# liuQuan98/EYOC

Measured on AMD Instinct MI355X. Metric: registered pairs/sec (30k-voxel KITTI pairs), higher is better.
Workload: dtype f32 (split16 products: fp32 storage/accumulation, 3 fp16 MFMAs on hi/lo-split operands per product); 1 GPU; 64 synthetic 30 cm KITTI-shaped pairs per step per GPU (mean 29894 voxels/cloud, ResUNetBN2C random-init, 5000-point NN, RANSAC 4000000 hypotheses/pair, planted inlier ratio 0.3, spconv math split16); parallelism=pairs sharded over 1 GPU(s), steps_in_flight=2

## Files before the change

eyoc_amd/_lib.py:

```python
from __future__ import annotations

import ctypes as C
import os
import threading

_HERE = os.path.dirname(os.path.abspath(__file__))
LIB_PATH = os.environ.get("EYOC_HIP_LIB") or os.path.join(_HERE, "lib", "libeyoc_hip.so")

MAX_LEVELS = 4
MAP_S1, MAP_DOWN, MAP_UP = 0, 1, 2


class MapsInfo(C.Structure):
    _fields_ = [("n_levels", C.c_int32), ("rows", C.c_int32 * MAX_LEVELS),
                ("pairs_s1", C.c_int64 * MAX_LEVELS), ("pairs_down", C.c_int64 * MAX_LEVELS),
                ("pairs_up", C.c_int64 * MAX_LEVELS), ("pairs_conv1", C.c_int64)]


class ModelDesc(C.Structure):
    _fields_ = [("in_channels", C.c_int32), ("out_channels", C.c_int32), ("conv1_kernel_size", C.c_int32),
                ("normalize_feature", C.c_int32), ("channels", C.c_int32 * 5), ("tr_channels", C.c_int32 * 5),
                ("bn_eps", C.c_float), ("expanded", C.c_int32)]


# ... 121 lines not shown
    "eyoc_model_layer_ms": (_i, [_vp, C.POINTER(C.c_float)]),
    "eyoc_model_timing_slot": (_i, [_vp, _i]),
    "eyoc_bn_workspace_bytes": (_sz, [_i, _i]),
    "eyoc_bn_train_forward": (_i, [_vp, _vp, _i, _i, _i, _vp, _vp, C.c_float, _i, _vp, _i, _vp, _vp, _sz, _vp]),
    "eyoc_bn_train_forward_running": (_i, [_vp, _vp, _i, _i, _i, _vp, _vp, C.c_float, _i, _vp, _i, _vp, _vp, _vp, C.c_float, _vp, _sz, _vp]),
    "eyoc_bn_train_backward": (_i, [_vp, _vp, _i, _vp, _i, _vp, _i, _i, _i, _vp, _vp, C.c_float, _vp, _i, _vp, _vp, _vp, _sz, _vp]),
    "eyoc_maps_gather_window": (_i, [_vp, _vp, _i, _vp, _i, _vp, _vp]),
    "eyoc_maps_gather_window_internal": (_i, [_vp, _vp, _i, _vp, _i, _vp, _vp]),
    "eyoc_knn_prefilter": (_i, [_vp, _i]),
    "eyoc_spconv_select_up_kernel": (_i, [_vp, _i]),
    "eyoc_spconv_upc_min_rows": (_i, [_vp, _i]),
    "eyoc_spconv_upc_tile_rows": (_i, [_i, _i]),
    "eyoc_spconv_upc_bytes": (_sz, [_i]),
    "eyoc_spconv_upc_build": (_i, [_vp, _vp, _i, _vp, _vp, _vp]),
    "eyoc_spconv_upc": (_i, [_vp, _vp, _vp, _i, _i, _vp, _i, _i, _vp, _i, _vp, _i, _vp, _i, _i, _vp, _vp]),
    "eyoc_spconv_select_conv1_kernel": (_i, [_vp, _i]),
    "eyoc_knn1": (_i, [_vp, _vp, _vp, _i, C.POINTER(C.c_int32), C.POINTER(C.c_int32), _i, _i, _vp, _vp, _vp]),
    "eyoc_pdist": (_i, [_vp, _vp, _i, _vp, _i, _i, _i, _vp, _vp]),
    "eyoc_kabsch_batched": (_i, [_vp, _vp, _vp, _vp, _i, _i, _vp, _vp]),
    "eyoc_irls_quad": (_i, [_vp, _vp, _vp, _vp, _i, _i, _vp, _vp]),
    "eyoc_ransac": (_i, [_vp, _vp, _vp, _vp, _i, C.POINTER(RansacParams), _vp, _vp]),
    "eyoc_maps_select_orders": (_i, [_vp, _i, _i]),
    "eyoc_ransac_select_pruning": (_i, [_vp, _i]),
    "eyoc_registration_accept_degenerate": (_i, [_vp, _i]),
    "eyoc_ransac_transform_store": (_i, [_vp, _i]),
    "eyoc_ransac_workspace_bytes": (_sz, [_vp, _i, _i, _i, _sz]),
    "eyoc_ransac_batched_ws": (_i, [_vp, _vp, _vp, _vp, C.POINTER(C.c_int32), C.POINTER(C.c_int32), _i,
                                    C.POINTER(RansacParams), _vp, _vp, _sz, _vp]),
    "eyoc_ransac_batched": (_i, [_vp, _vp, _vp, _vp, C.POINTER(C.c_int32), C.POINTER(C.c_int32), _i,
                                 C.POINTER(RansacParams), _vp, _vp]),
    "eyoc_sc2pcr_workspace_bytes": (_sz, [_i, C.POINTER(Sc2pcrParams)]),
    "eyoc_sc2pcr": (_i, [_vp, _vp, _vp, _i, C.POINTER(Sc2pcrParams), _vp, _vp, _vp, _sz, _vp]),
    "eyoc_sc2pcr_batched_workspace_bytes": (_sz, [_i, C.POINTER(Sc2pcrParams)]),
    "eyoc_sc2pcr_batched_workspace_bytes_n": (_sz, [_i, _i, C.POINTER(Sc2pcrParams)]),
    "eyoc_sc2pcr_set_shortlist_cap": (_i, [_vp, _i]),
    "eyoc_sc2pcr_set_dense_threshold": (_i, [_vp, _i]),
    "eyoc_sc2pcr_select_kernels": (_i, [_vp, _i]),
    "eyoc_sc2pcr_workspace_layout": (_i, [_i, C.POINTER(Sc2pcrParams), C.POINTER(Sc2pcrLayout)]),
    "eyoc_sc2pcr_batched": (_i, [_vp, _vp, _vp, C.POINTER(C.c_int32), _i, C.POINTER(Sc2pcrParams), _vp, _vp, _i, _vp, _sz,
                                 _vp]),
    "eyoc_icp_workspace_bytes": (_sz, [_i, _i, _i]),
    "eyoc_icp_batched": (_i, [_vp, _vp, _vp, C.POINTER(C.c_int32), C.POINTER(C.c_int32), _i, _vp, C.POINTER(IcpParams), _vp, _vp,
                              _vp, _sz, _vp]),
    "eyoc_icp_correspondences": (_i, [_vp, _vp, _vp, C.POINTER(C.c_int32), C.POINTER(C.c_int32), _i, _vp, C.c_double, _vp, _vp,
                                      _vp, _vp, _sz, _vp]),
}
# ... 139 lines not shown
```

eyoc_amd/csrc/common.h:

```cpp
#pragma once
#include <hip/hip_runtime.h>

#include <cstdarg>
#include <cstdint>
#include <cstdio>
#include <cstring>
#include <string>
#include <vector>

#include "../../include/eyoc_hip.h"

namespace eyoc {

void set_error(const char* fmt, ...);

#define EYOC_CHECK_HIP(expr)                                                               \
  do {                                                                                     \
    hipError_t _e = (expr);                                                                \
    if (_e != hipSuccess) {                                                                \
      eyoc::set_error("%s failed: %s (%s:%d)", #expr, hipGetErrorString(_e), __FILE__,    \
                      __LINE__);                                                           \
      return EYOC_ERR_HIP;                                                                 \
    }                                                                                      \
  } while (0)
// ... 49 lines not shown
  struct Knobs {
    int maps_order_min_rows = 65536;
    int maps_window_shift = 18;
    int maps_s1_order = 1, maps_down_order = 0;
    int maps_internal_order = -1;
    int maps_lazy_tables = 1, maps_fused_levels = 1;
    int knn_prefilter = 1;
    int fuse_tail = 2;
    int spconv_kernel = -1;
    int split16_kernel = 1;
    int up_kernel = 2;
    int s1_wide = 1;
    int st128_wide = 1;
    int down_kernel = 1;
    int upc_min_rows = 1 << 17;
    int conv1_kernel = 1;
    int st_group = 1;
    int st_variant = 1;
    int st_split_below = 1024;
    int st_cg_local = 1;
    int st_ksplit = 1;
    int ransac_store = 1 << 20;
    int ransac_prune = 2;
    int accept_degenerate = 0;
  } knobs;
};
inline const eyoc_ctx::Knobs& knobs_of(const eyoc_ctx* ctx) {
  static const eyoc_ctx::Knobs defaults;
  return ctx ? ctx->knobs : defaults;
}

namespace eyoc {

constexpr unsigned long long KEY_EMPTY = 0xFFFFFFFFFFFFFFFFull;
constexpr int COORD_BIAS = 1 << 17;
constexpr int VAL_UNSET = 0x7F7F7F7F;

struct HashTable {
  unsigned long long* keys;
  int* vals;
  unsigned int mask;
};

__host__ __device__ inline unsigned long long pack_key(int b, int x, int y, int z) {
  return ((unsigned long long)(unsigned)b << 54) |
         ((unsigned long long)((unsigned)(x + COORD_BIAS) & 0x3FFFFu) << 36) |
// ... 69 lines not shown
```

eyoc_amd/csrc/ransac.hip:

```cpp
#include "pose_math.h"

using namespace eyoc;

namespace {

__device__ inline void sample_pair(unsigned long long base, unsigned long long ctr, unsigned int n, unsigned int& i0,
                                   unsigned int& i1) {
  unsigned long long x = base + ctr;
  x = (x ^ (x >> 30)) * 0xBF58476D1CE4E5B9ull;
  x = (x ^ (x >> 27)) * 0x94D049BB133111EBull;
  x = x ^ (x >> 31);
  i0 = __umulhi((unsigned int)x, n);
  i1 = __umulhi((unsigned int)(x >> 32), n);
}

constexpr int CHUNK = 64;
struct PairArgs {
  int s0[CHUNK], n[CHUNK], t0[CHUNK];
  int pair0;
  float* rec;
  unsigned int seed;
  int H;
  float edge_sim, max_dist;
  int* n_surv;
  int* surv;
  int* cnts;
  unsigned int* rmse;
  double* xf;
  int cap_t;
  float* rec_sorted;
  float* rr_sorted;
  int* bucket_end;
  double* pmax;
  int count_bound;
};

__global__ void k_gather_targets(const float* __restrict__ src, const float* __restrict__ tgt,
                                 const long long* __restrict__ corr, PairArgs a) {
  const int c = blockIdx.y;
  const int s0 = a.s0[c], n = a.n[c];
  float* rec = a.rec;
  const int i = blockIdx.x * blockDim.x + threadIdx.x;
  if (i >= n) return;
  const long long j = a.t0[c] + corr[s0 + i];
  float* r = rec + (size_t)(s0 + i) * 6;
  r[0] = src[3 * (size_t)(s0 + i)]; r[1] = src[3 * (size_t)(s0 + i) + 1]; r[2] = src[3 * (size_t)(s0 + i) + 2];
  r[3] = tgt[3 * j]; r[4] = tgt[3 * j + 1]; r[5] = tgt[3 * j + 2];
}

__device__ inline bool sample_and_check_edges(const float* __restrict__ rec, unsigned int n, unsigned long long base,
                                              unsigned int h, double edge_sim, double s[4][3], double q[4][3]) {
  unsigned int idx[4];
  sample_pair(base, 2ull * h, n, idx[0], idx[1]);
  sample_pair(base, 2ull * h + 1, n, idx[2], idx[3]);
#pragma unroll
  for (int j = 0; j < 4; ++j) {
    const float2* r = reinterpret_cast<const float2*>(rec + (size_t)idx[j] * 6);
// ... 147 lines not shown
  const int* __restrict__ cand = a.cnts + (size_t)c * a.H;
  int* surv = a.surv + (size_t)c * a.H;
  const double edge_sim = (double)a.edge_sim, max_dist = (double)a.max_dist;
  for (int i = blockIdx.x * 256 + threadIdx.x; i < ncand; i += gridDim.x * 256) {
    const int h = cand[i];
    double s[4][3], q[4][3], R[3][3], t[3];
    sample_and_check_edges(rec, (unsigned)n, base, (unsigned)h, edge_sim, s, q);
    if (!fit_and_check_distance(s, q, max_dist, R, t)) continue;
    const int slot = atomicAdd(cnt, 1);
    surv[slot] = h;
    if (slot < a.cap_t) {
      double* x = a.xf + ((size_t)c * a.cap_t + slot) * 12;
#pragma unroll
      for (int k = 0; k < 3; ++k) {
        x[3 * k] = R[k][0]; x[3 * k + 1] = R[k][1]; x[3 * k + 2] = R[k][2];
        x[9 + k] = t[k];
      }
    }
  }
}

__device__ inline double thr2_of(float max_dist) { return (double)max_dist * (double)max_dist; }

constexpr int NBUCKET = 64;

__global__ __launch_bounds__(256) void k_bucket(PairArgs a) {
  __shared__ int hist[NBUCKET], start[NBUCKET];
  __shared__ double red[4];
  const int c = blockIdx.x;
  const int s0 = a.s0[c], n = a.n[c];
  const float* __restrict__ rec = a.rec + (size_t)s0 * 6;
  float* __restrict__ out = a.rec_sorted + (size_t)s0 * 6;
  int* bend = a.bucket_end + c * (NBUCKET + 1);
  const int ns = a.n_surv[c * CNT_STRIDE];
  if (threadIdx.x < NBUCKET) hist[threadIdx.x] = 0;
  __syncthreads();
  const bool have_ref = ns > 0;
  double R[9] = {1, 0, 0, 0, 1, 0, 0, 0, 1}, t[3] = {0, 0, 0};
  if (have_ref) {
    const double* x = a.xf + (size_t)c * a.cap_t * 12;
#pragma unroll
    for (int i = 0; i < 9; ++i) R[i] = x[i];
    t[0] = x[9]; t[1] = x[10]; t[2] = x[11];
  }
  const double inv_w = 1.0 / (double)a.max_dist;
  double pm = 0.0;
  int bkt[32];
#pragma unroll
  for (int u = 0; u < 32; ++u) {
    const int i = u * 256 + (int)threadIdx.x;
    bkt[u] = -1;
    if (i < n) {
      const float2* r = reinterpret_cast<const float2*>(rec + (size_t)i * 6);
      const float2 p0 = r[0], p1 = r[1], p2 = r[2];
      const double x = p0.x, y = p0.y, z = p1.x;
      const double dx = fma(R[0], x, fma(R[1], y, fma(R[2], z, t[0] - (double)p1.y)));
      const double dy = fma(R[3], x, fma(R[4], y, fma(R[5], z, t[1] - (double)p2.x)));
      const double dz = fma(R[6], x, fma(R[7], y, fma(R[8], z, t[2] - (double)p2.y)));
      const double d = sqrt(fma(dx, dx, fma(dy, dy, dz * dz)));
      const double q = d * inv_w;
      int b = have_ref ? (q < (double)(NBUCKET - 1) ? (int)q : NBUCKET - 1) : 0;
      if (!(q == q)) b = NBUCKET - 1;
      bkt[u] = b;
      atomicAdd(&hist[b], 1);
      pm = fmax(pm, sqrt(fma(x, x, fma(y, y, z * z))));
    }
  }
#pragma unroll
  for (int d = 32; d >= 1; d >>= 1) pm = fmax(pm, __shfl_xor(pm, d, 64));
  if ((threadIdx.x & 63) == 0) red[threadIdx.x >> 6] = pm;
  __syncthreads();
  if (threadIdx.x == 0) {
    int acc = 0;
    for (int b = 0; b < NBUCKET; ++b) { start[b] = acc; acc += hist[b]; bend[b] = acc; }
    bend[NBUCKET] = n;
    a.pmax[c] = fmax(fmax(red[0], red[1]), fmax(red[2], red[3]));
  }
  __syncthreads();
#pragma unroll
  for (int u = 0; u < 32; ++u) {
    const int i = u * 256 + (int)threadIdx.x;
    if (bkt[u] >= 0) {
      const int pos = atomicAdd(&start[bkt[u]], 1);
      const float2* r = reinterpret_cast<const float2*>(rec + (size_t)i * 6);
      float2* w = reinterpret_cast<float2*>(out + (size_t)pos * 6);
      const float2 p0 = r[0], p1 = r[1], p2 = r[2];
      w[0] = p0; w[1] = p1; w[2] = p2;
      const double x = p0.x, y = p0.y, z = p1.x;
      const double dx = fma(R[0], x, fma(R[1], y, fma(R[2], z, t[0] - (double)p1.y)));
      const double dy = fma(R[3], x, fma(R[4], y, fma(R[5], z, t[1] - (double)p2.x)));
      const double dz = fma(R[6], x, fma(R[7], y, fma(R[8], z, t[2] - (double)p2.y)));
      reinterpret_cast<float4*>(a.rr_sorted)[(size_t)s0 + pos] = make_float4((float)dx, (float)dy, (float)dz, 0.f);
    }
  }
}

constexpr int PPL = 4;

__global__ __launch_bounds__(256) void k_count_fp64(PairArgs a, const double* __restrict__ xf_all, int pruned) {
  const int c = blockIdx.y;
  const int s0 = a.s0[c], n = a.n[c];
  const float* __restrict__ rec = (pruned ? a.rec_sorted : a.rec) + (size_t)s0 * 6;
  const int lane = threadIdx.x & 63;
  const int wave = __builtin_amdgcn_readfirstlane((int)(threadIdx.x >> 6));
  const int ns_all = a.n_surv[c * CNT_STRIDE];
  const int ns = ns_all < a.cap_t ? ns_all : a.cap_t;
  const double thr2 = thr2_of(a.max_dist);
  const double* __restrict__ xf = xf_all + (size_t)c * a.cap_t * 12;
  const int* __restrict__ bend = a.bucket_end + c * (NBUCKET + 1);
  int* cnts = a.cnts + (size_t)c * a.H;
  int G = 64;
  while (G > 8 && (ns + G - 1) / G < (int)gridDim.x * 4) G >>= 1;
  const int n_groups = (ns + G - 1) / G;
  int best = 0;
  for (int grp = blockIdx.x * 4 + wave; grp < n_groups; grp += gridDim.x * 4) {
    const int sbase = grp * G;
    const int gs = min(G, ns - sbase);
    int hi = 0;
    if (lane < gs) {
      hi = n;
      if (pruned) {
        const double* __restrict__ T = xf + (size_t)(sbase + lane) * 12;
        double fr = 0.0, dt = 0.0;
#pragma unroll
        for (int i = 0; i < 9; ++i) { const double e = T[i] - xf[i]; fr = fma(e, e, fr); }
#pragma unroll
        for (int i = 9; i < 12; ++i) { const double e = T[i] - xf[i]; dt = fma(e, e, dt); }
        const double delta = (sqrt(fr) * a.pmax[c] + sqrt(dt)) * (1.0 + 1e-9) + 1e-9;
        const double q = ((double)a.max_dist + delta) / (double)a.max_dist;
        const int b = q < (double)(NBUCKET - 2) ? (int)q + 1 : NBUCKET;
        hi = bend[b < NBUCKET ? b : NBUCKET];
      }
    }
    int hi_max = hi;
#pragma unroll
    for (int d = 32; d >= 1; d >>= 1) hi_max = max(hi_max, __shfl_xor(hi_max, d, 64));
    hi_max = __builtin_amdgcn_readfirstlane(hi_max);
    int mycnt = 0;
    for (int i0 = 0; i0 < hi_max; i0 += 64 * PPL) {
      double x[PPL], y[PPL], z[PPL], qx[PPL], qy[PPL], qz[PPL];
#pragma unroll
      for (int u = 0; u < PPL; ++u) {
        const int i = i0 + u * 64 + lane;
        if (i < n) {
          const float2* r = reinterpret_cast<const float2*>(rec + (size_t)i * 6);
          const float2 p0 = r[0], p1 = r[1], p2 = r[2];
          x[u] = p0.x; y[u] = p0.y; z[u] = p1.x; qx[u] = p1.y; qy[u] = p2.x; qz[u] = p2.y;
        } else {
          x[u] = y[u] = z[u] = 0.0; qx[u] = qy[u] = qz[u] = 1e18;
        }
// ... 5 lines not shown
        const double r00 = T[0], r01 = T[1], r02 = T[2], r10 = T[3], r11 = T[4], r12 = T[5], r20 = T[6], r21 = T[7], r22 = T[8];
        const double t0 = T[9], t1 = T[10], t2 = T[11];
        int csum = 0;
#pragma unroll
        for (int u = 0; u < PPL; ++u) {
          const double dx = fma(r00, x[u], fma(r01, y[u], fma(r02, z[u], t0 - qx[u])));
          const double dy = fma(r10, x[u], fma(r11, y[u], fma(r12, z[u], t1 - qy[u])));
          const double dz = fma(r20, x[u], fma(r21, y[u], fma(r22, z[u], t2 - qz[u])));
          const double d2 = fma(dx, dx, fma(dy, dy, dz * dz));
          csum += __popcll(__ballot(d2 < thr2));
        }
        mycnt += lane == s ? csum : 0;
      }
    }
    if (lane < gs) cnts[sbase + lane] = mycnt;
    best = mycnt > best ? mycnt : best;
  }
#pragma unroll
  for (int d = 32; d >= 1; d >>= 1) best = max(best, __shfl_xor(best, d, 64));
  if (lane == 0 && best > 0) atomicMax(a.n_surv + c * CNT_STRIDE + 1, best);
}

typedef float f32x2 __attribute__((ext_vector_type(2)));
constexpr int PKP = 4;
constexpr int KC_RECORDS = 64 * 2 * PKP;

__device__ inline bool inlier_fp64(const float* __restrict__ rec, int i, const double* __restrict__ T, double thr2) {
  const float2* r = reinterpret_cast<const float2*>(rec + (size_t)i * 6);
  const float2 p0 = r[0], p1 = r[1], p2 = r[2];
  const double x = p0.x, y = p0.y, z = p1.x;
  const double dx = fma(T[0], x, fma(T[1], y, fma(T[2], z, T[9] - (double)p1.y)));
  const double dy = fma(T[3], x, fma(T[4], y, fma(T[5], z, T[10] - (double)p2.x)));
  const double dz = fma(T[6], x, fma(T[7], y, fma(T[8], z, T[11] - (double)p2.y)));
  return fma(dx, dx, fma(dy, dy, dz * dz)) < thr2;
}

__global__ __launch_bounds__(256) __attribute__((amdgpu_waves_per_eu(5, 5))) void k_count(PairArgs a, const double* __restrict__ xf_all) {
  __shared__ float4 deltas[4][64][3];
  const int c = blockIdx.y;
  const int s0 = a.s0[c], n = a.n[c];
  const float* __restrict__ rec = a.rec_sorted + (size_t)s0 * 6;
  const float4* __restrict__ rr = reinterpret_cast<const float4*>(a.rr_sorted) + s0;
  const int lane = threadIdx.x & 63;
  const int wave = __builtin_amdgcn_readfirstlane((int)(threadIdx.x >> 6));
  const int ns_all = a.n_surv[c * CNT_STRIDE];
  const int ns = ns_all < a.cap_t ? ns_all : a.cap_t;
  const double thr = (double)a.max_dist, thr2 = thr2_of(a.max_dist);
  const double* __restrict__ xf = xf_all + (size_t)c * a.cap_t * 12;
  const int* __restrict__ bend = a.bucket_end + c * (NBUCKET + 1);
  int* bestp = a.n_surv + c * CNT_STRIDE + 1;
  int pub_every = 1;
  while ((int)gridDim.x / pub_every > 64) pub_every <<= 1;
  const bool publisher = (blockIdx.x & (pub_every - 1)) == 0;
  int* cnts = a.cnts + (size_t)c * a.H;
  int G = 64;
  while (G > 8 && (ns + G - 1) / G < (int)gridDim.x * 4) G >>= 1;
  const int n_groups = (ns + G - 1) / G;
  int best = 0;
  for (int grp = blockIdx.x * 4 + wave; grp < n_groups; grp += gridDim.x * 4) {
    const int sbase = grp * G;
    const int gs = min(G, ns - sbase);
    int hi = 0;
    double m_dt = 0.0, m_dr = 0.0, m_t = 0.0, m_r = 1.0;
    if (lane < gs) {
      const double* __restrict__ T = xf + (size_t)(sbase + lane) * 12;
      double fr = 0.0, dt = 0.0;
      bool finite = true;
      float ef[12];
#pragma unroll
      for (int i = 0; i < 12; ++i) {
        const double v = T[i], r = xf[i], e = v - r;
        ef[i] = (float)e;
        finite = finite && fabs(v) < 1e300 && fabs(r) < 1e300;
        if (i < 9) { fr = fma(e, e, fr); m_dr = fmax(m_dr, fabs(e)); m_r = fmax(m_r, fmax(fabs(v), fabs(r))); }
        else { dt = fma(e, e, dt); m_dt = fmax(m_dt, fabs(e)); m_t = fmax(m_t, fmax(fabs(v), fabs(r))); }
      }
      if (!finite) m_t = 1e300;
#pragma unroll
      for (int k = 0; k < 3; ++k) deltas[wave][lane][k] = make_float4(ef[4 * k], ef[4 * k + 1], ef[4 * k + 2], ef[4 * k + 3]);
      const double delta = (sqrt(fr) * a.pmax[c] + sqrt(dt)) * (1.0 + 1e-9) + 1e-9;
      const double q = ((double)a.max_dist + delta) / (double)a.max_dist;
      const int b = q < (double)(NBUCKET - 2) ? (int)q + 1 : NBUCKET;
      hi = bend[b < NBUCKET ? b : NBUCKET];
    }
    int hi_max = hi;
#pragma unroll
    for (int d = 32; d >= 1; d >>= 1) hi_max = max(hi_max, __shfl_xor(hi_max, d, 64));
    hi_max = __builtin_amdgcn_readfirstlane(hi_max);
    int mycnt = 0;
    int known_next = a.count_bound ? __hip_atomic_load(bestp, __ATOMIC_RELAXED, __HIP_MEMORY_SCOPE_AGENT) : 0;
    for (int i0 = 0; i0 < hi_max; i0 += KC_RECORDS) {
      const int known = __builtin_amdgcn_readfirstlane(known_next);
      if (a.count_bound) known_next = __hip_atomic_load(bestp, __ATOMIC_RELAXED, __HIP_MEMORY_SCOPE_AGENT);
      const int ahead = hi - i0;
      const unsigned long long work = __ballot(lane < gs && ahead > 0 && mycnt + ahead >= known);
      if (!work) break;
      f32x2 x[PKP], y[PKP], z[PKP], rx[PKP], ry[PKP], rz[PKP];
      float mp = 0.f, mr = 0.f;
#pragma unroll
      for (int u = 0; u < PKP; ++u) {
        float v[2][6];
#pragma unroll
        for (int h = 0; h < 2; ++h) {
          const int i = i0 + (2 * u + h) * 64 + lane;
          if (i < n) {
            const float2* r = reinterpret_cast<const float2*>(rec + (size_t)i * 6);
            const float2 p0 = r[0], p1 = r[1];
            const float4 e = rr[i];
            v[h][0] = p0.x; v[h][1] = p0.y; v[h][2] = p1.x; v[h][3] = e.x; v[h][4] = e.y; v[h][5] = e.z;
#pragma unroll
            for (int k = 0; k < 6; ++k) {
              const float m = fabsf(v[h][k]) <= 3e38f ? fabsf(v[h][k]) : 3e38f;
              if (k < 3) mp = fmaxf(mp, m); else mr = fmaxf(mr, m);
            }
          } else {
            v[h][0] = v[h][1] = v[h][2] = 0.f; v[h][3] = v[h][4] = v[h][5] = 1e18f;
          }
        }
        x[u] = f32x2{v[0][0], v[1][0]}; y[u] = f32x2{v[0][1], v[1][1]}; z[u] = f32x2{v[0][2], v[1][2]};
// ... 51 lines not shown
          for (int u = 0; u < PKP; ++u)
#pragma unroll
            for (int h = 0; h < 2; ++h) {
              if (!amb[u][h]) continue;
              const int i = i0 + (2 * u + h) * 64 + lane;
              const bool in = ((amb[u][h] >> lane) & 1) && i < n && inlier_fp64(rec, i, T, thr2);
              csum += __popcll(__ballot(in));
            }
        }
        int m0_keep;
        asm volatile("s_mov_b32 %1, m0\n\ts_mov_b32 m0, %3\n\tv_writelane_b32 %0, %2, m0\n\ts_mov_b32 m0, %1"
                     : "+v"(blkcnt), "=&s"(m0_keep) : "s"(csum), "s"(s));
      }
      mycnt += blkcnt;
      if (a.count_bound && publisher) {
        int wm = mycnt;
#pragma unroll
        for (int d = 32; d >= 1; d >>= 1) wm = max(wm, __shfl_xor(wm, d, 64));
        if (lane == 0 && wm > known && wm > __hip_atomic_load(bestp, __ATOMIC_RELAXED, __HIP_MEMORY_SCOPE_AGENT)) atomicMax(bestp, wm);
      }
    }
    if (lane < gs) cnts[sbase + lane] = mycnt;
    best = mycnt > best ? mycnt : best;
  }
#pragma unroll
  for (int d = 32; d >= 1; d >>= 1) best = max(best, __shfl_xor(best, d, 64));
  if (lane == 0 && best > 0) atomicMax(a.n_surv + c * CNT_STRIDE + 1, best);
}

__device__ inline void sweep(const float* __restrict__ rec, int n, const double R[3][3], const double t[3], double thr2,
                             int lane, int& cnt_out, double& err2_out) {
  int cnt = 0;
  double err2 = 0;
  for (int i = lane; i < n; i += 64) {
    const float2* r = reinterpret_cast<const float2*>(rec + (size_t)i * 6);
    const float2 p0 = r[0], p1 = r[1], p2 = r[2];
    const double x = p0.x, y = p0.y, z = p1.x;
    const double dx = fma(R[0][0], x, fma(R[0][1], y, fma(R[0][2], z, t[0] - (double)p1.y)));
    const double dy = fma(R[1][0], x, fma(R[1][1], y, fma(R[1][2], z, t[1] - (double)p2.x)));
    const double dz = fma(R[2][0], x, fma(R[2][1], y, fma(R[2][2], z, t[2] - (double)p2.y)));
    const double d2 = fma(dx, dx, fma(dy, dy, dz * dz));
    if (d2 < thr2) { ++cnt; err2 += d2; }
  }
#pragma unroll
  for (int d = 32; d >= 1; d >>= 1) cnt += __shfl_down(cnt, d, 64);
  cnt_out = cnt;
// ... 124 lines not shown
  l.bytes = align_up(l.off_pm + (size_t)chunk * 8);
  return l;
}
int ransac_pick_chunk(int n_pairs, int total, int H, size_t budget, int store) {
  int chunk = n_pairs < CHUNK ? n_pairs : CHUNK;
  while (chunk > 1 && ransac_layout(chunk, total, H, store).bytes > budget) chunk >>= 1;
  return chunk;
}

int ransac_run(eyoc_ctx* ctx, const float* src_dev, const float* tgt_dev, const int64_t* corr_tgt_dev, const int32_t* seg_src_host,
               const int32_t* seg_tgt_host, int n_pairs, const eyoc_ransac_params* p, eyoc_ransac_result* results_dev, char* sc,
               int chunk, int max_n, int store, hipStream_t st) {
  const int H = p->max_iteration;
  const int total = seg_src_host[n_pairs];
  const int cap_t = ransac_cap_t(H, store);
  const RansacLayout l = ransac_layout(chunk, total, H, store);
  PairArgs a;
  a.rec = (float*)(sc + l.off_rec); a.seed = p->seed; a.H = H; a.edge_sim = p->edge_similarity; a.max_dist = p->max_distance;
  a.n_surv = (int*)(sc + l.off_cnt); a.surv = (int*)(sc + l.off_surv); a.cnts = (int*)(sc + l.off_cnts);
  a.rmse = (unsigned int*)(sc + l.off_rmse); a.xf = (double*)(sc + l.off_xf); a.cap_t = cap_t;
  a.rec_sorted = (float*)(sc + l.off_rs); a.rr_sorted = (float*)(sc + l.off_rr); a.bucket_end = (int*)(sc + l.off_be); a.pmax = (double*)(sc + l.off_pm);
  const int pruned = ctx->knobs.ransac_prune && max_n <= 8192 ? 1 : 0;
  const int want_bound = ctx->knobs.ransac_prune >= 2 ? 1 : 0;
  const bool in_lds = max_n <= LDS_RECORDS;
  const size_t lds_bytes = in_lds ? (size_t)max_n * 24 : 0;
  if (in_lds) {
    if (!ctx->ransac_attr_set) {
      EYOC_CHECK_HIP(hipFuncSetAttribute(reinterpret_cast<const void*>(k_generate<true>), hipFuncAttributeMaxDynamicSharedMemorySize,
                                         LDS_RECORDS * 24));
      ctx->ransac_attr_set = true;
    }
  }
  for (int p0 = 0; p0 < n_pairs; p0 += chunk) {
    const int nc = n_pairs - p0 < chunk ? n_pairs - p0 : chunk;
    a.pair0 = p0;
    a.count_bound = want_bound && nc >= 32 ? 1 : 0;
    int chunk_max = 0;
    for (int c = 0; c < CHUNK; ++c) {
      const int b = p0 + (c < nc ? c : 0);
      a.s0[c] = seg_src_host[b]; a.n[c] = seg_src_host[b + 1] - seg_src_host[b]; a.t0[c] = seg_tgt_host[b];
      chunk_max = a.n[c] > chunk_max ? a.n[c] : chunk_max;
    }
    EYOC_CHECK_HIP(hipMemsetAsync(a.n_surv, 0, (size_t)nc * CNT_STRIDE * 4, st));
    hipLaunchKernelGGL(k_gather_targets, dim3(cdiv(chunk_max, 256), nc), dim3(256), 0, st, src_dev, tgt_dev,
                       (const long long*)corr_tgt_dev, a);
    const int gen_blocks = GEN_BLOCKS_TOTAL / nc > GEN_BLOCKS_MIN ? GEN_BLOCKS_TOTAL / nc : GEN_BLOCKS_MIN;
    if (in_lds) hipLaunchKernelGGL(k_generate<true>, dim3(gen_blocks, nc), dim3(GEN_THREADS), lds_bytes, st, a);
    else hipLaunchKernelGGL(k_generate<false>, dim3(gen_blocks, nc), dim3(GEN_THREADS), 0, st, a);
    hipLaunchKernelGGL(k_fit, dim3(2048 / nc > 8 ? 2048 / nc : 8, nc), dim3(256), 0, st, a);
    if (pruned) hipLaunchKernelGGL(k_bucket, dim3(nc), dim3(256), 0, st, a);
    constexpr int KC_BLOCKS = 4096;
    if (pruned) hipLaunchKernelGGL(k_count, dim3(KC_BLOCKS / nc, nc), dim3(256), 0, st, a, (const double*)a.xf);
    else hipLaunchKernelGGL(k_count_fp64, dim3(KC_BLOCKS / nc, nc), dim3(256), 0, st, a, (const double*)a.xf, pruned);
    if (H > cap_t) hipLaunchKernelGGL(k_count_overflow, dim3(256, nc), dim3(256), 0, st, a);
    hipLaunchKernelGGL(k_rmse, dim3(64, nc), dim3(256), 0, st, a);
    hipLaunchKernelGGL(k_select, dim3(nc), dim3(1024), 0, st, a, results_dev);
  }
  EYOC_CHECK_HIP(hipGetLastError());
  return EYOC_OK;
}

int ransac_validate(const float* src_dev, const float* tgt_dev, const int64_t* corr_tgt_dev, const int32_t* seg_src_host,
                    const int32_t* seg_tgt_host, int n_pairs, const eyoc_ransac_params* p, eyoc_ransac_result* results_dev, int* max_n) {
  EYOC_REQUIRE(src_dev && tgt_dev && corr_tgt_dev && seg_src_host && seg_tgt_host && p && results_dev, EYOC_ERR_INVALID,
               "eyoc_ransac_batched: NULL argument");
  EYOC_REQUIRE(n_pairs >= 1, EYOC_ERR_INVALID, "eyoc_ransac_batched: n_pairs %d", n_pairs);
  EYOC_REQUIRE(p->max_iteration >= 1, EYOC_ERR_INVALID, "eyoc_ransac: max_iteration %d", p->max_iteration);
  *max_n = 0;
  for (int b = 0; b < n_pairs; ++b) {
    const int n = seg_src_host[b + 1] - seg_src_host[b];
    EYOC_REQUIRE(n >= 4, EYOC_ERR_INVALID, "eyoc_ransac: need at least 4 correspondences, got %d (pair %d)", n, b);
    *max_n = n > *max_n ? n : *max_n;
  }
  return EYOC_OK;
}
// ... 48 lines not shown
  return EYOC_OK;
}

}

extern "C" int eyoc_registration_accept_degenerate(eyoc_ctx* ctx, int on) {
  if (!ctx) return -1;
  const int prev = ctx->knobs.accept_degenerate;
  if (on == 0 || on == 1) ctx->knobs.accept_degenerate = on;
  return prev;
}

extern "C" int eyoc_ransac_transform_store(eyoc_ctx* ctx, int survivors) {
  if (!ctx) return -1;
  const int prev = ctx->knobs.ransac_store;
  if (survivors >= 1) ctx->knobs.ransac_store = survivors;
  return prev;
}

extern "C" int eyoc_ransac_select_pruning(eyoc_ctx* ctx, int on) {
  if (!ctx) return -1;
  const int prev = ctx->knobs.ransac_prune;
  if (on >= 0 && on <= 2) ctx->knobs.ransac_prune = on;
  return prev;
}

extern "C" size_t eyoc_ransac_workspace_bytes(const eyoc_ctx* ctx, int n_pairs, int total_corr, int max_iteration, size_t budget_bytes) {
  if (n_pairs < 1 || total_corr < 0 || max_iteration < 1) return 0;
  const int store = knobs_of(ctx).ransac_store;
  const int chunk = ransac_pick_chunk(n_pairs, total_corr, max_iteration, budget_bytes ? budget_bytes : ~(size_t)0, store);
  return ransac_layout(chunk, total_corr, max_iteration, store).bytes;
}

extern "C" int eyoc_ransac_batched_ws(eyoc_ctx* ctx, const float* src_dev, const float* tgt_dev, const int64_t* corr_tgt_dev,
                                      const int32_t* seg_src_host, const int32_t* seg_tgt_host, int n_pairs,
                                      const eyoc_ransac_params* p, eyoc_ransac_result* results_dev, void* workspace_dev,
                                      size_t workspace_bytes, void* stream) {
  EYOC_REQUIRE(ctx && workspace_dev, EYOC_ERR_INVALID, "eyoc_ransac_batched_ws: NULL argument");
  EYOC_REQUIRE(((uintptr_t)workspace_dev & 255) == 0, EYOC_ERR_INVALID, "eyoc_ransac_batched_ws: workspace must be 256-byte aligned");
  int rc = ransac_split(ctx, seg_src_host, seg_tgt_host, n_pairs, p, results_dev, (hipStream_t)stream,
                        [&](const int32_t* ss, const int32_t* stt, int np, const eyoc_ransac_params* q, eyoc_ransac_result* r) {
                          return eyoc_ransac_batched_ws(ctx, src_dev, tgt_dev, corr_tgt_dev, ss, stt, np, q, r, workspace_dev,
                                                        workspace_bytes, stream);
                        });
  if (rc <= 0) return rc;
  int max_n = 0;
// ... 55 lines not shown
```

eyoc_amd/registration.py:

```python
from __future__ import annotations

import ctypes as C
from dataclasses import dataclass

import numpy as np
import torch

from . import _lib
from .eval import _cuda_f32, knn1_segmented
from .transform_estimation import transform


@dataclass
class RegistrationResult:
    transformation: np.ndarray
    fitness: float
    inlier_rmse: float
    inliers: int = 0
    best_hypothesis: int = -1
    survivors: int = 0
    status: int = 0
    correspondence_set: np.ndarray | None = None
    iterations: int = 0


def ransac_from_correspondences(src, tgt, corr_tgt, max_correspondence_distance, max_iteration=4000000, seed=0,
                                edge_similarity=0.9, as_device_result=False):
    s = _cuda_f32(src)
    t = _cuda_f32(tgt, s.device)
    c = corr_tgt.to(s.device, torch.int64).contiguous()
    n = s.shape[0]
    res = ransac_batched_from_correspondences(s, t, c, [0, n], [0, 0], max_correspondence_distance, max_iteration, seed,
                                              edge_similarity)[0]
    if as_device_result:
        return res
    return decode_ransac_result(res, n)


def ransac_batched_from_correspondences(src, tgt, corr_tgt, seg_src, seg_tgt, max_correspondence_distance,
                                        max_iteration=4000000, seed=0, edge_similarity=0.9, workspace_budget=None):
    s = _cuda_f32(src)
    t = _cuda_f32(tgt, s.device)
    c = corr_tgt.to(s.device, torch.int64).contiguous()
    P = len(seg_src) - 1
    ss = (C.c_int32 * (P + 1))(*[int(v) for v in seg_src])
    st = (C.c_int32 * (P + 1))(*[int(v) for v in seg_tgt])
    p = _lib.RansacParams(float(max_correspondence_distance), float(edge_similarity), int(max_iteration), int(seed))
    res = torch.empty((P, C.sizeof(_lib.RansacResult)), dtype=torch.uint8, device=s.device)
    lib = _lib.load()
    with torch.cuda.device(s.device):
        budget = int(workspace_budget) if workspace_budget else _ransac_budget(s.device)
        ws = _lib.workspace(lib.eyoc_ransac_workspace_bytes(_lib.ctx(s.device.index), P, int(seg_src[-1]), int(max_iteration), budget), s.device)
        _lib.check(lib.eyoc_ransac_batched_ws(_lib.ctx(s.device.index), _lib.ptr(s), _lib.ptr(t), _lib.ptr(c), ss, st, P,
                                              C.byref(p), _lib.ptr(res), _lib.ptr(ws), ws.numel(), _lib.stream_ptr()),
                   "eyoc_ransac_batched_ws")
    return res


def _ransac_budget(device) -> int:
    free, _ = torch.cuda.mem_get_info(device)
    cached = torch.cuda.memory_reserved(device) - torch.cuda.memory_allocated(device)
    return max(min((free + cached) // 4, 16 << 30), 1)


def decode_ransac_result(res: torch.Tensor, n: int) -> RegistrationResult:
    r = _lib.RansacResult.from_buffer_copy(res.cpu().numpy().tobytes())
    T = np.array(list(r.T), np.float64).reshape(4, 4)
    return RegistrationResult(T, r.inliers / max(n, 1), float(r.inlier_rmse), int(r.inliers),
                              int(r.best_hypothesis), int(r.survivors))


def registration_ransac_based_on_feature_matching(source, target, source_feature, target_feature,
                                                  mutual_filter=False, max_correspondence_distance=0.3,
                                                  estimation_method=None, ransac_n=4, checkers=None,
                                                  criteria=(4000000, 0.999), seed=0, edge_similarity=0.9):
    if mutual_filter:
        raise NotImplementedError("mutual_filter=True is not used by the reference path")
    if ransac_n != 4:
        raise NotImplementedError("ransac_n must be 4 (scripts/test_kitti.py:174)")
# ... 105 lines not shown
```

include/eyoc_hip.h:

```cpp
#ifndef EYOC_HIP_H
#define EYOC_HIP_H

#include <stddef.h>
#include <stdint.h>

#ifdef __cplusplus
extern "C" {
#endif

typedef struct eyoc_ctx eyoc_ctx;
typedef struct eyoc_maps eyoc_maps;
typedef struct eyoc_model eyoc_model;

typedef enum {
  EYOC_OK = 0,
  EYOC_ERR_INVALID = -1,
  EYOC_ERR_HIP = -2,
  EYOC_ERR_WORKSPACE = -3,
  EYOC_ERR_DUPLICATE = -4,
  EYOC_ERR_RANGE = -5
} eyoc_status;

#define EYOC_MAX_LEVELS 4
#define EYOC_VERSION 111
// ... 200 lines not shown
  int32_t max_iteration;
  uint32_t seed;
} eyoc_ransac_params;

typedef struct {
  float T[16];
  int32_t inliers;
  int32_t best_hypothesis;
  int32_t survivors;
  float inlier_rmse;
} eyoc_ransac_result;

int eyoc_ransac(eyoc_ctx* ctx, const float* src_dev, const float* tgt_dev, const int64_t* corr_tgt_dev,
                int n, const eyoc_ransac_params* params, eyoc_ransac_result* result_dev, void* stream);
size_t eyoc_ransac_workspace_bytes(const eyoc_ctx* ctx, int n_pairs, int total_corr, int max_iteration, size_t budget_bytes);
int eyoc_ransac_batched_ws(eyoc_ctx* ctx, const float* src_dev, const float* tgt_dev, const int64_t* corr_tgt_dev,
                           const int32_t* seg_src_host, const int32_t* seg_tgt_host, int n_pairs,
                           const eyoc_ransac_params* params, eyoc_ransac_result* results_dev, void* workspace_dev,
                           size_t workspace_bytes, void* stream);
int eyoc_ransac_batched(eyoc_ctx* ctx, const float* src_dev, const float* tgt_dev, const int64_t* corr_tgt_dev,
                        const int32_t* seg_src_host, const int32_t* seg_tgt_host, int n_pairs,
                        const eyoc_ransac_params* params, eyoc_ransac_result* results_dev, void* stream);
int eyoc_ransac_select_pruning(eyoc_ctx* ctx, int on);
int eyoc_registration_accept_degenerate(eyoc_ctx* ctx, int on);
int eyoc_ransac_transform_store(eyoc_ctx* ctx, int survivors);

typedef struct {
  float inlier_threshold, d_thre, ratio, nms_radius;
  int32_t num_iterations, max_points, k1, k2;
} eyoc_sc2pcr_params;
size_t eyoc_sc2pcr_workspace_bytes(int n, const eyoc_sc2pcr_params* params);
int eyoc_sc2pcr(eyoc_ctx* ctx, const float* src_dev, const float* tgt_dev, int n,
                const eyoc_sc2pcr_params* params, float* T_dev, float* fitness_dev,
                void* workspace_dev, size_t workspace_bytes, void* stream);
size_t eyoc_sc2pcr_batched_workspace_bytes(int max_n, const eyoc_sc2pcr_params* params);
size_t eyoc_sc2pcr_batched_workspace_bytes_n(int max_n, int n_pairs, const eyoc_sc2pcr_params* params);
int eyoc_sc2pcr_batched(eyoc_ctx* ctx, const float* src_dev, const float* tgt_dev, const int32_t* seg_host,
                        int n_pairs, const eyoc_sc2pcr_params* params, float* T_dev, float* fitness_dev,
                        int fitness_stride, void* workspace_dev, size_t workspace_bytes, void* stream);
int eyoc_sc2pcr_set_shortlist_cap(eyoc_ctx* ctx, int cap);
int eyoc_sc2pcr_set_dense_threshold(eyoc_ctx* ctx, int x);
int eyoc_sc2pcr_select_kernels(eyoc_ctx* ctx, int legacy_bits);
typedef struct {
  int32_t n, words, n_seed, k1, k2, n_part, col_chunk, reserved;
  int64_t csr_cap;
  uint64_t total;
// ... 34 lines not shown
```

Before: 3195 pairs/s.

## Order RANSAC inlier counting by best reference hypothesis and point-norm bins

Result: faster. 3232 pairs/s (median of 6 runs) (+1.2%).

```diff
diff --git a/eyoc_amd/_lib.py b/eyoc_amd/_lib.py
--- a/eyoc_amd/_lib.py
+++ b/eyoc_amd/_lib.py
@@ -167,6 +167,7 @@
     "eyoc_ransac": (_i, [_vp, _vp, _vp, _vp, _i, C.POINTER(RansacParams), _vp, _vp]),
     "eyoc_maps_select_orders": (_i, [_vp, _i, _i]),
     "eyoc_ransac_select_pruning": (_i, [_vp, _i]),
+    "eyoc_ransac_select_count_order": (_i, [_vp, _i]),
     "eyoc_registration_accept_degenerate": (_i, [_vp, _i]),
     "eyoc_ransac_transform_store": (_i, [_vp, _i]),
     "eyoc_ransac_workspace_bytes": (_sz, [_vp, _i, _i, _i, _sz]),
diff --git a/eyoc_amd/csrc/common.h b/eyoc_amd/csrc/common.h
--- a/eyoc_amd/csrc/common.h
+++ b/eyoc_amd/csrc/common.h
@@ -95,6 +95,7 @@
     int st_ksplit = 1;
     int ransac_store = 1 << 20;
     int ransac_prune = 2;
+    int ransac_count_order = 1;
     int accept_degenerate = 0;
   } knobs;
 };
diff --git a/eyoc_amd/csrc/ransac.hip b/eyoc_amd/csrc/ransac.hip
--- a/eyoc_amd/csrc/ransac.hip
+++ b/eyoc_amd/csrc/ransac.hip
@@ -33,6 +33,7 @@
   int* bucket_end;
   double* pmax;
   int count_bound;
+  int count_order;
 };
 
 __global__ void k_gather_targets(const float* __restrict__ src, const float* __restrict__ tgt,
@@ -226,10 +227,56 @@
 
 __device__ inline double thr2_of(float max_dist) { return (double)max_dist * (double)max_dist; }
 
+__device__ inline bool inlier_fp64(const float* __restrict__ rec, int i, const double* __restrict__ T, double thr2) {
+  const float2* r = reinterpret_cast<const float2*>(rec + (size_t)i * 6);
+  const float2 p0 = r[0], p1 = r[1], p2 = r[2];
+  const double x = p0.x, y = p0.y, z = p1.x;
+  const double dx = fma(T[0], x, fma(T[1], y, fma(T[2], z, T[9] - (double)p1.y)));
+  const double dy = fma(T[3], x, fma(T[4], y, fma(T[5], z, T[10] - (double)p2.x)));
+  const double dz = fma(T[6], x, fma(T[7], y, fma(T[8], z, T[11] - (double)p2.y)));
+  return fma(dx, dx, fma(dy, dy, dz * dz)) < thr2;
+}
+
 constexpr int NBUCKET = 64;
-
+constexpr int NBIN = 8;
+#ifndef KC_REF_CAND
+#define KC_REF_CAND 64
+#endif
+constexpr int REF_CAND = KC_REF_CAND;
+constexpr int CNT_REF = 3, CNT_WORK = 4;
+
+__device__ inline int ref_slot(const int* __restrict__ cnt_line) {
+  const int key = cnt_line[CNT_REF];
+  return key > 0 ? 63 - ((key - 1) & 63) : 0;
+}
+
+__global__ __launch_bounds__(256) void k_ref(PairArgs a) {
+  static_assert(REF_CAND <= 64, "k_ref's key: 6 bits of slot under the count (at most 8192 on bucketed records)");
+  const int c = blockIdx.y;
+  const int lane = threadIdx.x & 63;
+  const int s = blockIdx.x * 4 + (int)(threadIdx.x >> 6);
+  int* cnt = a.n_surv + c * CNT_STRIDE;
+  const int ns = cnt[0];
+  const int cand = min(min(ns, a.cap_t), REF_CAND);
+  if (s >= cand || cand < 2) return;
+  const int n = a.n[c];
+  const float* __restrict__ rec = a.rec + (size_t)a.s0[c] * 6;
+  const double* __restrict__ T = a.xf + ((size_t)c * a.cap_t + s) * 12;
+  const double thr2 = thr2_of(a.max_dist);
+  int k = 0;
+  for (int i = lane; i < n; i += 64) k += inlier_fp64(rec, i, T, thr2) ? 1 : 0;
+#pragma unroll
+  for (int d = 32; d >= 1; d >>= 1) k += __shfl_xor(k, d, 64);
+  if (lane == 0) {
+    atomicMax(cnt + CNT_REF, ((k << 6) | (63 - s)) + 1);
+    atomicMax(cnt + 1, k);
+  }
+}
+
+template <bool ORDER>
 __global__ __launch_bounds__(256) void k_bucket(PairArgs a) {
-  __shared__ int hist[NBUCKET], start[NBUCKET];
+  constexpr int NB = ORDER ? NBIN : 1, NCELL = NBUCKET * NB;
+  __shared__ int hist[NCELL], start[NCELL];
   __shared__ double red[4];
   const int c = blockIdx.x;
   const int s0 = a.s0[c], n = a.n[c];
@@ -237,12 +284,12 @@
   float* __restrict__ out = a.rec_sorted + (size_t)s0 * 6;
   int* bend = a.bucket_end + c * (NBUCKET + 1);
   const int ns = a.n_surv[c * CNT_STRIDE];
-  if (threadIdx.x < NBUCKET) hist[threadIdx.x] = 0;
+  for (int i = threadIdx.x; i < NCELL; i += 256) hist[i] = 0;
   __syncthreads();
   const bool have_ref = ns > 0;
   double R[9] = {1, 0, 0, 0, 1, 0, 0, 0, 1}, t[3] = {0, 0, 0};
   if (have_ref) {
-    const double* x = a.xf + (size_t)c * a.cap_t * 12;
+    const double* x = a.xf + ((size_t)c * a.cap_t + ref_slot(a.n_surv + c * CNT_STRIDE)) * 12;
 #pragma unroll
     for (int i = 0; i < 9; ++i) R[i] = x[i];
     t[0] = x[9]; t[1] = x[10]; t[2] = x[11];
@@ -250,6 +297,7 @@
   const double inv_w = 1.0 / (double)a.max_dist;
   double pm = 0.0;
   int bkt[32];
+  float pn[ORDER ? 32 : 1];
 #pragma unroll
   for (int u = 0; u < 32; ++u) {
     const int i = u * 256 + (int)threadIdx.x;
@@ -266,19 +314,46 @@
       int b = have_ref ? (q < (double)(NBUCKET - 1) ? (int)q : NBUCKET - 1) : 0;
       if (!(q == q)) b = NBUCKET - 1;
       bkt[u] = b;
-      atomicAdd(&hist[b], 1);
-      pm = fmax(pm, sqrt(fma(x, x, fma(y, y, z * z))));
+      const double norm = sqrt(fma(x, x, fma(y, y, z * z)));
+      if constexpr (ORDER) pn[u] = (float)norm;
+      else atomicAdd(&hist[b], 1);
+      pm = fmax(pm, norm);
     }
   }
 #pragma unroll
   for (int d = 32; d >= 1; d >>= 1) pm = fmax(pm, __shfl_xor(pm, d, 64));
   if ((threadIdx.x & 63) == 0) red[threadIdx.x >> 6] = pm;
   __syncthreads();
-  if (threadIdx.x == 0) {
-    int acc = 0;
-    for (int b = 0; b < NBUCKET; ++b) { start[b] = acc; acc += hist[b]; bend[b] = acc; }
-    bend[NBUCKET] = n;
-    a.pmax[c] = fmax(fmax(red[0], red[1]), fmax(red[2], red[3]));
+  pm = fmax(fmax(red[0], red[1]), fmax(red[2], red[3]));
+  if constexpr (ORDER) {
+    const float scale = pm > 0.0 && pm < 1e30 ? (float)((double)NBIN / pm) : 0.f;
+#pragma unroll
+    for (int u = 0; u < 32; ++u)
+      if (bkt[u] >= 0) {
+        const float f = pn[u] * scale;
+        const int bin = f >= 0.f && f < (float)NBIN ? (int)f : NBIN - 1;
+        bkt[u] = bkt[u] * NBIN + (NBIN - 1 - bin);
+        atomicAdd(&hist[bkt[u]], 1);
+      }
+    __syncthreads();
+  }
+  if (threadIdx.x < 64) {
+    static_assert(NBUCKET == 64, "one lane per bucket");
+    const int b = threadIdx.x;
+    int tot = 0;
+#pragma unroll
+    for (int k = 0; k < NB; ++k) tot += hist[b * NB + k];
+    int incl = tot;
+#pragma unroll
+    for (int d = 1; d < 64; d <<= 1) {
+      const int v = __shfl_up(incl, d, 64);
+      if (b >= d) incl += v;
+    }
+    int acc = incl - tot;
+#pragma unroll
+    for (int k = 0; k < NB; ++k) { start[b * NB + k] = acc; acc += hist[b * NB + k]; }
+    bend[b] = incl;
+    if (b == 0) { bend[NBUCKET] = n; a.pmax[c] = pm; }
   }
   __syncthreads();
 #pragma unroll
@@ -311,6 +386,7 @@
   const int ns = ns_all < a.cap_t ? ns_all : a.cap_t;
   const double thr2 = thr2_of(a.max_dist);
   const double* __restrict__ xf = xf_all + (size_t)c * a.cap_t * 12;
+  const double* __restrict__ xref = xf + (size_t)ref_slot(a.n_surv + c * CNT_STRIDE) * 12;
   const int* __restrict__ bend = a.bucket_end + c * (NBUCKET + 1);
   int* cnts = a.cnts + (size_t)c * a.H;
   int G = 64;
@@ -327,9 +403,9 @@
         const double* __restrict__ T = xf + (size_t)(sbase + lane) * 12;
         double fr = 0.0, dt = 0.0;
 #pragma unroll
-        for (int i = 0; i < 9; ++i) { const double e = T[i] - xf[i]; fr = fma(e, e, fr); }
-#pragma unroll
-        for (int i = 9; i < 12; ++i) { const double e = T[i] - xf[i]; dt = fma(e, e, dt); }
+        for (int i = 0; i < 9; ++i) { const double e = T[i] - xref[i]; fr = fma(e, e, fr); }
+#pragma unroll
+        for (int i = 9; i < 12; ++i) { const double e = T[i] - xref[i]; dt = fma(e, e, dt); }
         const double delta = (sqrt(fr) * a.pmax[c] + sqrt(dt)) * (1.0 + 1e-9) + 1e-9;
         const double q = ((double)a.max_dist + delta) / (double)a.max_dist;
         const int b = q < (double)(NBUCKET - 2) ? (int)q + 1 : NBUCKET;
@@ -381,20 +457,13 @@
 }
 
 typedef float f32x2 __attribute__((ext_vector_type(2)));
-constexpr int PKP = 4;
-constexpr int KC_RECORDS = 64 * 2 * PKP;
-
-__device__ inline bool inlier_fp64(const float* __restrict__ rec, int i, const double* __restrict__ T, double thr2) {
-  const float2* r = reinterpret_cast<const float2*>(rec + (size_t)i * 6);
-  const float2 p0 = r[0], p1 = r[1], p2 = r[2];
-  const double x = p0.x, y = p0.y, z = p1.x;
-  const double dx = fma(T[0], x, fma(T[1], y, fma(T[2], z, T[9] - (double)p1.y)));
-  const double dy = fma(T[3], x, fma(T[4], y, fma(T[5], z, T[10] - (double)p2.x)));
-  const double dz = fma(T[6], x, fma(T[7], y, fma(T[8], z, T[11] - (double)p2.y)));
-  return fma(dx, dx, fma(dy, dy, dz * dz)) < thr2;
-}
-
+
+#ifndef KC_PKP_ORDERED
+#define KC_PKP_ORDERED 2
+#endif
+template <int PKP>
 __global__ __launch_bounds__(256) __attribute__((amdgpu_waves_per_eu(5, 5))) void k_count(PairArgs a, const double* __restrict__ xf_all) {
+  constexpr int KC_RECORDS = 64 * 2 * PKP;
   __shared__ float4 deltas[4][64][3];
   const int c = blockIdx.y;
   const int s0 = a.s0[c], n = a.n[c];
@@ -406,6 +475,7 @@
   const int ns = ns_all < a.cap_t ? ns_all : a.cap_t;
   const double thr = (double)a.max_dist, thr2 = thr2_of(a.max_dist);
   const double* __restrict__ xf = xf_all + (size_t)c * a.cap_t * 12;
+  const double* __restrict__ xref = xf + (size_t)ref_slot(a.n_surv + c * CNT_STRIDE) * 12;
   const int* __restrict__ bend = a.bucket_end + c * (NBUCKET + 1);
   int* bestp = a.n_surv + c * CNT_STRIDE + 1;
   int pub_every = 1;
@@ -428,7 +498,7 @@
       float ef[12];
 #pragma unroll
       for (int i = 0; i < 12; ++i) {
-        const double v = T[i], r = xf[i], e = v - r;
+        const double v = T[i], r = xref[i], e = v - r;
         ef[i] = (float)e;
         finite = finite && fabs(v) < 1e300 && fabs(r) < 1e300;
         if (i < 9) { fr = fma(e, e, fr); m_dr = fmax(m_dr, fabs(e)); m_r = fmax(m_r, fmax(fabs(v), fabs(r))); }
@@ -447,6 +517,7 @@
     for (int d = 32; d >= 1; d >>= 1) hi_max = max(hi_max, __shfl_xor(hi_max, d, 64));
     hi_max = __builtin_amdgcn_readfirstlane(hi_max);
     int mycnt = 0;
+    int sweeps = 0;
     int known_next = a.count_bound ? __hip_atomic_load(bestp, __ATOMIC_RELAXED, __HIP_MEMORY_SCOPE_AGENT) : 0;
     for (int i0 = 0; i0 < hi_max; i0 += KC_RECORDS) {
       const int known = __builtin_amdgcn_readfirstlane(known_next);
@@ -454,6 +525,7 @@
       const int ahead = hi - i0;
       const unsigned long long work = __ballot(lane < gs && ahead > 0 && mycnt + ahead >= known);
       if (!work) break;
+      sweeps += __popcll(work);
       f32x2 x[PKP], y[PKP], z[PKP], rx[PKP], ry[PKP], rz[PKP];
       float mp = 0.f, mr = 0.f;
 #pragma unroll
@@ -551,6 +623,7 @@
     }
     if (lane < gs) cnts[sbase + lane] = mycnt;
     best = mycnt > best ? mycnt : best;
+    if (lane == 0 && sweeps) atomicAdd(a.n_surv + c * CNT_STRIDE + CNT_WORK, sweeps * PKP);
   }
 #pragma unroll
   for (int d = 32; d >= 1; d >>= 1) best = max(best, __shfl_xor(best, d, 64));
@@ -721,6 +794,7 @@
   a.rec_sorted = (float*)(sc + l.off_rs); a.rr_sorted = (float*)(sc + l.off_rr); a.bucket_end = (int*)(sc + l.off_be); a.pmax = (double*)(sc + l.off_pm);
   const int pruned = ctx->knobs.ransac_prune && max_n <= 8192 ? 1 : 0;
   const int want_bound = ctx->knobs.ransac_prune >= 2 ? 1 : 0;
+  const int want_order = pruned && ctx->knobs.ransac_count_order ? 1 : 0;
   const bool in_lds = max_n <= LDS_RECORDS;
   const size_t lds_bytes = in_lds ? (size_t)max_n * 24 : 0;
   if (in_lds) {
@@ -734,6 +808,7 @@
     const int nc = n_pairs - p0 < chunk ? n_pairs - p0 : chunk;
     a.pair0 = p0;
     a.count_bound = want_bound && nc >= 32 ? 1 : 0;
+    a.count_order = want_order && a.count_bound ? 1 : 0;
     int chunk_max = 0;
     for (int c = 0; c < CHUNK; ++c) {
       const int b = p0 + (c < nc ? c : 0);
@@ -747,9 +822,15 @@
     if (in_lds) hipLaunchKernelGGL(k_generate<true>, dim3(gen_blocks, nc), dim3(GEN_THREADS), lds_bytes, st, a);
     else hipLaunchKernelGGL(k_generate<false>, dim3(gen_blocks, nc), dim3(GEN_THREADS), 0, st, a);
     hipLaunchKernelGGL(k_fit, dim3(2048 / nc > 8 ? 2048 / nc : 8, nc), dim3(256), 0, st, a);
-    if (pruned) hipLaunchKernelGGL(k_bucket, dim3(nc), dim3(256), 0, st, a);
+    if (a.count_order) {
+      hipLaunchKernelGGL(k_ref, dim3(REF_CAND / 4, nc), dim3(256), 0, st, a);
+      hipLaunchKernelGGL(k_bucket<true>, dim3(nc), dim3(256), 0, st, a);
+    } else if (pruned) {
+      hipLaunchKernelGGL(k_bucket<false>, dim3(nc), dim3(256), 0, st, a);
+    }
     constexpr int KC_BLOCKS = 4096;
-    if (pruned) hipLaunchKernelGGL(k_count, dim3(KC_BLOCKS / nc, nc), dim3(256), 0, st, a, (const double*)a.xf);
+    if (a.count_order) hipLaunchKernelGGL(k_count<KC_PKP_ORDERED>, dim3(KC_BLOCKS / nc, nc), dim3(256), 0, st, a, (const double*)a.xf);
+    else if (pruned) hipLaunchKernelGGL(k_count<4>, dim3(KC_BLOCKS / nc, nc), dim3(256), 0, st, a, (const double*)a.xf);
     else hipLaunchKernelGGL(k_count_fp64, dim3(KC_BLOCKS / nc, nc), dim3(256), 0, st, a, (const double*)a.xf, pruned);
     if (H > cap_t) hipLaunchKernelGGL(k_count_overflow, dim3(256, nc), dim3(256), 0, st, a);
     hipLaunchKernelGGL(k_rmse, dim3(64, nc), dim3(256), 0, st, a);
@@ -844,6 +925,13 @@
   if (!ctx) return -1;
   const int prev = ctx->knobs.ransac_prune;
   if (on >= 0 && on <= 2) ctx->knobs.ransac_prune = on;
+  return prev;
+}
+
+extern "C" int eyoc_ransac_select_count_order(eyoc_ctx* ctx, int on) {
+  if (!ctx) return -1;
+  const int prev = ctx->knobs.ransac_count_order;
+  if (on == 0 || on == 1) ctx->knobs.ransac_count_order = on;
   return prev;
 }
 
diff --git a/eyoc_amd/registration.py b/eyoc_amd/registration.py
--- a/eyoc_amd/registration.py
+++ b/eyoc_amd/registration.py
@@ -38,7 +38,7 @@
 
 
 def ransac_batched_from_correspondences(src, tgt, corr_tgt, seg_src, seg_tgt, max_correspondence_distance,
-                                        max_iteration=4000000, seed=0, edge_similarity=0.9, workspace_budget=None):
+                                        max_iteration=4000000, seed=0, edge_similarity=0.9, workspace_budget=None, _work=None):
     s = _cuda_f32(src)
     t = _cuda_f32(tgt, s.device)
     c = corr_tgt.to(s.device, torch.int64).contiguous()
@@ -54,7 +54,20 @@
         _lib.check(lib.eyoc_ransac_batched_ws(_lib.ctx(s.device.index), _lib.ptr(s), _lib.ptr(t), _lib.ptr(c), ss, st, P,
                                               C.byref(p), _lib.ptr(res), _lib.ptr(ws), ws.numel(), _lib.stream_ptr()),
                    "eyoc_ransac_batched_ws")
+        if _work is not None:
+            single = ws.numel() >= lib.eyoc_ransac_workspace_bytes(_lib.ctx(s.device.index), P, int(seg_src[-1]), int(max_iteration), 0) and P <= 64
+            if not single:
+                raise _lib.EyocError("the scorer's work counter is per launch chunk: this call ran in several (raise workspace_budget, at most 64 pairs)")
+            _work.append(ws[:P * 256].view(torch.int32).view(P, 64)[:, 4].clone())
     return res
+
+
+def ransac_batched_count_work(src, tgt, corr_tgt, seg_src, seg_tgt, max_correspondence_distance, max_iteration=4000000, seed=0,
+                              edge_similarity=0.9, workspace_budget=None):
+    work = []
+    res = ransac_batched_from_correspondences(src, tgt, corr_tgt, seg_src, seg_tgt, max_correspondence_distance, max_iteration, seed,
+                                              edge_similarity, workspace_budget, _work=work)
+    return res, work[0]
 
 
 def _ransac_budget(device) -> int:
diff --git a/include/eyoc_hip.h b/include/eyoc_hip.h
--- a/include/eyoc_hip.h
+++ b/include/eyoc_hip.h
@@ -246,6 +246,7 @@
                         const int32_t* seg_src_host, const int32_t* seg_tgt_host, int n_pairs,
                         const eyoc_ransac_params* params, eyoc_ransac_result* results_dev, void* stream);
 int eyoc_ransac_select_pruning(eyoc_ctx* ctx, int on);
+int eyoc_ransac_select_count_order(eyoc_ctx* ctx, int on);
 int eyoc_registration_accept_degenerate(eyoc_ctx* ctx, int on);
 int eyoc_ransac_transform_store(eyoc_ctx* ctx, int survivors);
 
```
